# ApsaraDB/galaxysql

Hardware: NVIDIA H100
Metric: joined+aggregated rows/sec; achieved HBM GB/s vs peak, at 1/2/4/8 H100 (higher is better)
Workload: dtype int64

## Files before the change

galaxysql_b200/csrc/join_fast.cuh:

```cuda
#pragma once

#include <cub/block/block_scan.cuh>
#include <cub/device/device_scan.cuh>

#include "common.cuh"

namespace fj {

constexpr unsigned long long KEY_EMPTY = 0x8000000000000000ULL;
constexpr int THREADS = 512;
constexpr int RPT = 4;
constexpr int TILE = THREADS * RPT;
constexpr int MAX_WORDS = 4;
constexpr int MAX_P = 1024;
constexpr int MAX_DISP = 4096;
enum { FL_SENTINEL = 0, FL_DUP = 1, FL_DISP = 2, FL_NULLOUT = 3, FL_SPILL = 4, FL_COUNT = 5 };

struct Layout {
    int32_t nwords, ncols, key_col, key_i32;
    int32_t word[GSQL_MAX_COLS];
    int32_t half[GSQL_MAX_COLS];
};

static bool make_layout(const int32_t *types, int ncols, int key_col, Layout *L) {
    memset(L, 0, sizeof(*L));
    L->ncols = ncols;
    L->key_col = key_col;
    L->key_i32 = types[key_col] == GSQL_T_INT32;
    int next = 1;
    int open_word = -1;
    for (int c = 0; c < ncols; c++) {
        if (c == key_col) {
            L->word[c] = 0;
            L->half[c] = L->key_i32 ? 0 : 2;
            continue;
        }
        if (types[c] == GSQL_T_INT32) {
            if (open_word >= 0) {
                L->word[c] = open_word;
                L->half[c] = 1;
                open_word = -1;
            } else {
                L->word[c] = next;
                L->half[c] = 0;
                open_word = next++;
            }
        } else {
            L->word[c] = next++;
            L->half[c] = 2;
        }
    }
    L->nwords = next;
    return next <= MAX_WORDS;
}

__device__ __forceinline__ uint64_t key_hash(unsigned long long k) { return (k ^ (k >> 32)) * 0x9E3779B97F4A7C15ULL; }

template <int W>
__device__ __forceinline__ void pack_row(const DColSet &cols, const Layout &L, int64_t r, unsigned long long (&w)[W]) {
#pragma unroll
    for (int i = 0; i < W; i++) w[i] = 0;
#pragma unroll 1
    for (int c = 0; c < L.ncols; c++) {
        const DCol &col = cols.c[c];
        unsigned long long v;
        if (col.type == GSQL_T_INT32) {
            int x = ld_stream_4(reinterpret_cast<const int *>(col.data) + r);
            v = c == L.key_col ? (unsigned long long)(long long)x : (unsigned long long)(unsigned)x;
        } else {
            v = (unsigned long long)ld_stream_8(reinterpret_cast<const long long *>(col.data) + r);
        }
        int wi = L.word[c];
        if (L.half[c] == 1) v <<= 32;
#pragma unroll
        for (int i = 0; i < W; i++)
            if (i == wi) w[i] |= v;
    }
}

template <int W, int NC>
__device__ __forceinline__ void pack_tile_nc(const DColSet &cols, const Layout &L, int64_t base, int64_t limit, unsigned long long (&w)[RPT][W]) {
    unsigned long long v[NC > 0 ? NC : 1][RPT];
#pragma unroll
    for (int c = 0; c < NC; c++) {
        const DCol &col = cols.c[c];
        const bool is32 = col.type == GSQL_T_INT32;
#pragma unroll
        for (int k = 0; k < RPT; k++) {
            int64_t r = base + k * THREADS;
            v[c][k] = 0;
            if (r < limit) {
                if (is32) v[c][k] = (unsigned long long)(unsigned)ld_stream_4(reinterpret_cast<const int *>(col.data) + r);
                else v[c][k] = (unsigned long long)ld_stream_8(reinterpret_cast<const long long *>(col.data) + r);
            }
        }
    }
#pragma unroll
    for (int k = 0; k < RPT; k++)
#pragma unroll
        for (int i = 0; i < W; i++) w[k][i] = 0;
#pragma unroll
    for (int c = 0; c < NC; c++) {
        const bool sext = c == L.key_col && cols.c[c].type == GSQL_T_INT32;
        const int wi = L.word[c];
        const int sh = L.half[c] == 1 ? 32 : 0;
#pragma unroll
        for (int k = 0; k < RPT; k++) {
            unsigned long long vv = sext ? (unsigned long long)(long long)(int)(unsigned)v[c][k] : v[c][k];
            vv <<= sh;
#pragma unroll
            for (int i = 0; i < W; i++)
                if (i == wi) w[k][i] |= vv;
        }
    }
}

template <int W>
__device__ __forceinline__ void pack_tile_generic(const DColSet &cols, const Layout &L, int64_t base, int64_t limit, unsigned long long (&w)[RPT][W]) {
#pragma unroll
    for (int k = 0; k < RPT; k++)
#pragma unroll
        for (int i = 0; i < W; i++) w[k][i] = 0;
#pragma unroll 1
    for (int c = 0; c < L.ncols; c++) {
        const DCol &col = cols.c[c];
        const bool is32 = col.type == GSQL_T_INT32, iskey = c == L.key_col;
        const int wi = L.word[c];
        const int sh = L.half[c] == 1 ? 32 : 0;
        unsigned long long v[RPT];
#pragma unroll
        for (int k = 0; k < RPT; k++) {
            int64_t r = base + k * THREADS;
            v[k] = 0;
            if (r < limit) {
                if (is32) {
                    int x = ld_stream_4(reinterpret_cast<const int *>(col.data) + r);
                    v[k] = iskey ? (unsigned long long)(long long)x : (unsigned long long)(unsigned)x;
                } else {
                    v[k] = (unsigned long long)ld_stream_8(reinterpret_cast<const long long *>(col.data) + r);
                }
            }
        }
#pragma unroll
        for (int k = 0; k < RPT; k++) {
            unsigned long long vv = v[k] << sh;
#pragma unroll
            for (int i = 0; i < W; i++)
                if (i == wi) w[k][i] |= vv;
        }
    }
}

template <int W>
__device__ __forceinline__ void pack_tile(const DColSet &cols, const Layout &L, int64_t base, int64_t limit, unsigned long long (&w)[RPT][W]) {
    switch (L.ncols) {
    case 1: pack_tile_nc<W, 1>(cols, L, base, limit, w); break;
    case 2: pack_tile_nc<W, 2>(cols, L, base, limit, w); break;
    case 3: pack_tile_nc<W, 3>(cols, L, base, limit, w); break;
    case 4: pack_tile_nc<W, 4>(cols, L, base, limit, w); break;
    default: pack_tile_generic<W>(cols, L, base, limit, w); break;
    }
}

__device__ __forceinline__ unsigned long long load_key(const DCol &col, int64_t r) {
    if (col.type == GSQL_T_INT32) return (unsigned long long)(long long)ld_stream_4(reinterpret_cast<const int *>(col.data) + r);
    return (unsigned long long)ld_stream_8(reinterpret_cast<const long long *>(col.data) + r);
}

__device__ __forceinline__ unsigned int part_of(uint64_t h, int P) { return __umulhi((unsigned int)(h >> 32), (unsigned int)P); }

struct PartGeom {
    int64_t rows, chunk;
    int32_t P, nblocks;
};

template <int NT>
__global__ void __launch_bounds__(NT) k_fj_hist(DCol keycol, PartGeom g, int64_t *__restrict__ hist, int32_t *flags) {
    extern __shared__ unsigned int sh_hist[];
    for (int i = threadIdx.x; i < g.P; i += NT) sh_hist[i] = 0;
    __syncthreads();
    int64_t r0 = (int64_t)blockIdx.x * g.chunk;
    int64_t r1 = r0 + g.chunk < g.rows ? r0 + g.chunk : g.rows;
    bool sentinel = false;
    for (int64_t t0 = r0; t0 < r1; t0 += NT * RPT) {
        unsigned long long key[RPT];
#pragma unroll
        for (int k = 0; k < RPT; k++) {
            int64_t r = t0 + k * NT + threadIdx.x;
            key[k] = r < r1 ? load_key(keycol, r) : 0;
        }
#pragma unroll
        for (int k = 0; k < RPT; k++) {
            int64_t r = t0 + k * NT + threadIdx.x;
            if (r < r1) {
                sentinel |= key[k] == KEY_EMPTY;
                atomicAdd(&sh_hist[part_of(key_hash(key[k]), g.P)], 1u);
            }
        }
    }
    if (sentinel) flags[FL_SENTINEL] = 1;
    __syncthreads();
    for (int i = threadIdx.x; i < g.P; i += NT) hist[(int64_t)i * g.nblocks + blockIdx.x] = sh_hist[i];
}

__device__ __forceinline__ void cp_async_4(void *smem_dst, const void *gsrc) {
    asm volatile("cp.async.ca.shared.global [%0], [%1], 4;" ::"r"((uint32_t)__cvta_generic_to_shared(smem_dst)), "l"(gsrc) : "memory");
}
__device__ __forceinline__ void cp_async_8(void *smem_dst, const void *gsrc) {
    asm volatile("cp.async.ca.shared.global [%0], [%1], 8;" ::"r"((uint32_t)__cvta_generic_to_shared(smem_dst)), "l"(gsrc) : "memory");
}
__device__ __forceinline__ void cp_async_16(void *smem_dst, const void *gsrc) {
    asm volatile("cp.async.cg.shared.global [%0], [%1], 16;" ::"r"((uint32_t)__cvta_generic_to_shared(smem_dst)), "l"(gsrc) : "memory");
}
__device__ __forceinline__ void cp_async_16_hint(void *smem_dst, const void *gsrc, uint64_t pol) {
    asm volatile("cp.async.cg.shared.global.L2::cache_hint [%0], [%1], 16, %2;" ::"r"((uint32_t)__cvta_generic_to_shared(smem_dst)), "l"(gsrc), "l"(pol)
                 : "memory");
}
__device__ __forceinline__ void cp_async_commit() { asm volatile("cp.async.commit_group;" ::: "memory"); }
template <int N>
__device__ __forceinline__ void cp_async_wait() { asm volatile("cp.async.wait_group %0;" ::"n"(N) : "memory"); }

__device__ __forceinline__ uint32_t smem_u32(const void *p) { return (uint32_t)__cvta_generic_to_shared(p); }
__device__ __forceinline__ void mbar_init(unsigned long long *bar, int count) {
    asm volatile("mbarrier.init.shared::cta.b64 [%0], %1;" ::"r"(smem_u32(bar)), "r"(count) : "memory");
}
__device__ __forceinline__ void mbar_expect_tx(unsigned long long *bar, uint32_t bytes) {
    asm volatile("mbarrier.arrive.expect_tx.shared::cta.b64 _, [%0], %1;" ::"r"(smem_u32(bar)), "r"(bytes) : "memory");
}
__device__ __forceinline__ void mbar_wait(unsigned long long *bar, uint32_t parity) {
    uint32_t done = 0;
    while (!done)
        asm volatile("{\n\t.reg .pred p;\n\tmbarrier.try_wait.parity.shared::cta.b64 p, [%1], %2;\n\tselp.u32 %0, 1, 0, p;\n\t}"
                     : "=r"(done) : "r"(smem_u32(bar)), "r"(parity) : "memory");
}
__device__ __forceinline__ uint64_t l2_policy_evict_first() {
    uint64_t pol;
    asm volatile("createpolicy.fractional.L2::evict_first.b64 %0, 1.0;" : "=l"(pol));
    return pol;
}
__device__ __forceinline__ void tma_load_1d(void *smem_dst, const void *gsrc, uint32_t bytes, unsigned long long *bar, uint64_t pol) {
    asm volatile("cp.async.bulk.shared::cluster.global.mbarrier::complete_tx::bytes.L2::cache_hint [%0], [%1], %2, [%3], %4;" ::"r"(smem_u32(smem_dst)),
                 "l"(gsrc), "r"(bytes), "r"(smem_u32(bar)), "l"(pol)
                 : "memory");
}

template <bool FULL>
__device__ __forceinline__ void tile_prefetch(const DColSet &cols, const Layout &L, int64_t t0, int n_tile, unsigned char *buf) {
    const unsigned tid = threadIdx.x;
    unsigned char *sp = buf + tid * 4u;
#pragma unroll 1
    for (int c = 0; c < L.ncols; c++) {
        const DCol &col = cols.c[c];
        if (col.type == GSQL_T_INT32) {
            const int *gp = reinterpret_cast<const int *>(col.data) + t0 + tid;
#pragma unroll
            for (int k = 0; k < RPT; k++)
                if (FULL || (int)(k * THREADS + tid) < n_tile) cp_async_4(sp + k * THREADS * 4, gp + k * THREADS);
            sp += TILE * 4;
        } else {
            const long long *gp = reinterpret_cast<const long long *>(col.data) + t0 + tid;
            unsigned char *sp8 = sp + tid * 4u;
#pragma unroll
            for (int k = 0; k < RPT; k++)
                if (FULL || (int)(k * THREADS + tid) < n_tile) cp_async_8(sp8 + k * THREADS * 8, gp + k * THREADS);
            sp += TILE * 8;
        }
    }
    cp_async_commit();
}

template <int W, bool FULL>
__device__ __forceinline__ void pack_tile_smem(const DColSet &cols, const Layout &L, int n_tile, const unsigned char *buf,
                                               unsigned long long (&w)[RPT][W]) {
#pragma unroll
    for (int k = 0; k < RPT; k++)
#pragma unroll
        for (int i = 0; i < W; i++) w[k][i] = 0;
    const unsigned tid = threadIdx.x;
    const unsigned char *sp = buf + tid * 4u;
#pragma unroll 1
    for (int c = 0; c < L.ncols; c++) {
        const bool is32 = cols.c[c].type == GSQL_T_INT32, iskey = c == L.key_col;
        const int wi = L.word[c];
        const int sh = L.half[c] == 1 ? 32 : 0;
        unsigned long long v[RPT];
        if (is32) {
#pragma unroll
            for (int k = 0; k < RPT; k++) {
                int x = (FULL || (int)(k * THREADS + tid) < n_tile) ? *reinterpret_cast<const int *>(sp + k * THREADS * 4) : 0;
                v[k] = iskey ? (unsigned long long)(long long)x : (unsigned long long)(unsigned)x;
            }
            sp += TILE * 4;
        } else {
            const unsigned char *sp8 = sp + tid * 4u;
#pragma unroll
            for (int k = 0; k < RPT; k++)
                v[k] = (FULL || (int)(k * THREADS + tid) < n_tile) ? *reinterpret_cast<const unsigned long long *>(sp8 + k * THREADS * 8) : 0ULL;
            sp += TILE * 8;
        }
#pragma unroll
        for (int i = 0; i < W; i++)
            if (i == wi) {
#pragma unroll
                for (int k = 0; k < RPT; k++) w[k][i] |= v[k] << sh;
            }
    }
}

template <int W, bool PIPE>
__global__ void __launch_bounds__(THREADS, 2) k_fj_scatter(const __grid_constant__ DColSet cols, const __grid_constant__ Layout L, PartGeom g,
                                                        const int64_t *__restrict__ offs, unsigned long long *__restrict__ out) {
    extern __shared__ __align__(16) unsigned char smem_raw[];
    unsigned long long *stage = reinterpret_cast<unsigned long long *>(smem_raw);
    unsigned long long *cur = stage + (size_t)TILE * W;
    unsigned long long *delta = cur + g.P;
    unsigned int *hist = reinterpret_cast<unsigned int *>(delta + g.P);
    unsigned int *start = hist + g.P;
    unsigned short *spid = reinterpret_cast<unsigned short *>(start + g.P);
    unsigned char *inbuf = reinterpret_cast<unsigned char *>(spid + TILE);
    typedef cub::BlockScan<unsigned int, THREADS> BlockScan;
    __shared__ typename BlockScan::TempStorage scan_tmp;

    for (int p = threadIdx.x; p < g.P; p += THREADS) {
        cur[p] = (unsigned long long)offs[(int64_t)p * g.nblocks + blockIdx.x];
        hist[p] = 0;
    }
    __syncthreads();
    int64_t r0 = (int64_t)blockIdx.x * g.chunk;
    int64_t r1 = r0 + g.chunk < g.rows ? r0 + g.chunk : g.rows;
    if (PIPE && r0 < r1) {
        if (r1 - r0 >= TILE) tile_prefetch<true>(cols, L, r0, TILE, inbuf);
        else tile_prefetch<false>(cols, L, r0, (int)(r1 - r0), inbuf);
    }
    int it = 0;
    for (int64_t t0 = r0; t0 < r1; t0 += TILE, it++) {
        unsigned long long w[RPT][W];
        unsigned int pid[RPT], rank[RPT];
        const int n_tile = (int)(r1 - t0 < TILE ? r1 - t0 : TILE);
        const bool full = n_tile == TILE;
        if (PIPE) {
            const int64_t left = r1 - (t0 + TILE);
            unsigned char *nbuf = inbuf + (size_t)((it + 1) & 1) * TILE * W * 8;
            if (left >= TILE) tile_prefetch<true>(cols, L, t0 + TILE, TILE, nbuf);
            else if (left > 0) tile_prefetch<false>(cols, L, t0 + TILE, (int)left, nbuf);
            else cp_async_commit();
            cp_async_wait<1>();
            const unsigned char *cbuf = inbuf + (size_t)(it & 1) * TILE * W * 8;
            if (full) pack_tile_smem<W, true>(cols, L, n_tile, cbuf, w);
            else pack_tile_smem<W, false>(cols, L, n_tile, cbuf, w);
        } else {
            pack_tile<W>(cols, L, t0 + threadIdx.x, r1, w);
        }
        if (full) {
#pragma unroll
            for (int k = 0; k < RPT; k++) {
                pid[k] = part_of(key_hash(w[k][0]), g.P);
                rank[k] = atomicAdd(&hist[pid[k]], 1u);
            }
        } else {
#pragma unroll
            for (int k = 0; k < RPT; k++) {
                pid[k] = 0xffffffffu;
                if ((int)(k * THREADS + threadIdx.x) < n_tile) {
                    pid[k] = part_of(key_hash(w[k][0]), g.P);
                    rank[k] = atomicAdd(&hist[pid[k]], 1u);
                }
            }
        }
        __syncthreads();
        {
            constexpr int IPT = MAX_P / THREADS;
            unsigned int v[IPT];
#pragma unroll
            for (int i = 0; i < IPT; i++) {
                int p = threadIdx.x * IPT + i;
                v[i] = p < g.P ? hist[p] : 0;
            }
            BlockScan(scan_tmp).ExclusiveSum(v, v);
#pragma unroll
            for (int i = 0; i < IPT; i++) {
                int p = threadIdx.x * IPT + i;
                if (p < g.P) {
                    start[p] = v[i];
                    unsigned long long c = cur[p];
                    delta[p] = c - v[i];
                    cur[p] = c + hist[p];
                    hist[p] = 0;
                }
            }
        }
        __syncthreads();
#pragma unroll
        for (int k = 0; k < RPT; k++) {
            if (full || pid[k] != 0xffffffffu) {
                unsigned int pos = start[pid[k]] + rank[k];
                if (W == 2) {
                    int4 v;
                    v.x = (int)(unsigned)w[k][0]; v.y = (int)(unsigned)(w[k][0] >> 32);
                    v.z = (int)(unsigned)w[k][W - 1]; v.w = (int)(unsigned)(w[k][W - 1] >> 32);
                    *reinterpret_cast<int4 *>(stage + (size_t)pos * 2) = v;
                } else {
#pragma unroll
                    for (int i = 0; i < W; i++) stage[(size_t)pos * W + i] = w[k][i];
                }
                spid[pos] = (unsigned short)pid[k];
            }
        }
        __syncthreads();
#pragma unroll
        for (int k = 0; k < RPT; k++) {
            const int i = k * THREADS + threadIdx.x;
            if (full || i < n_tile) {
                unsigned long long dst = delta[spid[i]] + (unsigned)i;
                if (W == 2) {
                    st_stream_16(out + dst * 2, *reinterpret_cast<const int4 *>(stage + (size_t)i * 2));
                } else {
#pragma unroll
                    for (int j = 0; j < W; j++) st_stream_8(out + dst * W + j, (long long)stage[(size_t)i * W + j]);
                }
            }
        }
        __syncthreads();
    }
}

template <int W>
__global__ void __launch_bounds__(THREADS, 2) k_fj_scatter_direct(const __grid_constant__ DColSet cols, const __grid_constant__ Layout L, PartGeom g,
                                                               const int64_t *__restrict__ offs, unsigned long long *__restrict__ out) {
    extern __shared__ __align__(16) unsigned char smem_raw[];
    unsigned long long *base = reinterpret_cast<unsigned long long *>(smem_raw);
    unsigned int *cnt = reinterpret_cast<unsigned int *>(base + g.P);
    for (int p = threadIdx.x; p < g.P; p += THREADS) {
        base[p] = (unsigned long long)offs[(int64_t)p * g.nblocks + blockIdx.x];
        cnt[p] = 0;
    }
    __syncthreads();
    const int64_t r0 = (int64_t)blockIdx.x * g.chunk;
    const int64_t r1 = r0 + g.chunk < g.rows ? r0 + g.chunk : g.rows;
    for (int64_t t0 = r0; t0 < r1; t0 += TILE) {
        unsigned long long w[RPT][W];
        pack_tile<W>(cols, L, t0 + threadIdx.x, r1, w);
#pragma unroll
        for (int k = 0; k < RPT; k++) {
            if (t0 + k * THREADS + threadIdx.x >= r1) continue;
            const unsigned int pid = part_of(key_hash(w[k][0]), g.P);
            const unsigned long long dst = base[pid] + atomicAdd(&cnt[pid], 1u);
            if (W == 2) {
                int4 v;
                v.x = (int)(unsigned)w[k][0]; v.y = (int)(unsigned)(w[k][0] >> 32);
                v.z = (int)(unsigned)w[k][W - 1]; v.w = (int)(unsigned)(w[k][W - 1] >> 32);
                *reinterpret_cast<int4 *>(out + dst * 2) = v;
            } else {
#pragma unroll
                for (int i = 0; i < W; i++) out[dst * W + i] = w[k][i];
            }
        }
    }
}

static size_t scatter_smem_bytes(int W, int P, bool pipe) {
    return (size_t)TILE * W * 8 + (size_t)P * 8 * 2 + (size_t)P * 4 * 2 + (size_t)TILE * 2 + (pipe ? (size_t)2 * TILE * W * 8 : 0);
}

constexpr int SM_THREADS = 1024;
__host__ __device__ constexpr int sm_rpt_max(int W) { return W == 1 ? 8 : W == 2 ? 6 : W == 3 ? 4 : 3; }

static size_t scatter_sm_smem_bytes(int W, int P, int rpt) {
    const size_t T = (size_t)SM_THREADS * rpt;
    return T * W * 8 * 2 + (size_t)P * (8 * 3 + 4 * 3) + T * 2;
}

struct Regions {
    unsigned long long *fill;
    int64_t cap;
    int32_t K;
};

template <int W>
__global__ void __launch_bounds__(SM_THREADS, 1) k_fj_scatter_sm(const __grid_constant__ DColSet cols, const __grid_constant__ Layout L, PartGeom g,
                                                                 int rpt, const int64_t *__restrict__ offs, Regions RG,
                                                                 unsigned long long *__restrict__ out, int32_t *flags) {
    constexpr int R = sm_rpt_max(W);
    const int T = SM_THREADS * rpt;
    extern __shared__ __align__(128) unsigned char smem_raw[];
    unsigned long long *stage = reinterpret_cast<unsigned long long *>(smem_raw);
    unsigned char *inbuf = reinterpret_cast<unsigned char *>(stage + (size_t)T * W);
    unsigned long long *cur = reinterpret_cast<unsigned long long *>(inbuf + (size_t)T * W * 8);
    unsigned long long *delta = cur + g.P;
    unsigned long long *delta2 = delta + g.P;
    unsigned int *hist = reinterpret_cast<unsigned int *>(delta2 + g.P);
    unsigned int *start = hist + g.P;
    unsigned int *split = start + g.P;
    unsigned short *spid = reinterpret_cast<unsigned short *>(split + g.P);
    __shared__ __align__(8) unsigned long long bar;
    __shared__ int spill;
    typedef cub::BlockScan<unsigned int, SM_THREADS, cub::BLOCK_SCAN_WARP_SCANS> BlockScan;
    __shared__ typename BlockScan::TempStorage scan_tmp;
    const int tid = threadIdx.x, lane = tid & 31, warp = tid >> 5;

    uint32_t bulk_bytes = 0, my_off = 0, off = 0;
    bool my_bulk = false;
    for (int c = 0; c < L.ncols; c++) {
        const uint32_t bytes = (uint32_t)T * (cols.c[c].type == GSQL_T_INT32 ? 4u : 8u);
        const bool aligned = ((uintptr_t)cols.c[c].data & 15) == 0;
        if (c == warp) { my_off = off; my_bulk = aligned; }
        off += bytes;
        if (aligned) bulk_bytes += bytes;
    }
    const bool issuer = lane == 0 && warp < L.ncols && my_bulk;
    uint64_t pol = 0;
    if (issuer) pol = l2_policy_evict_first();

    if (tid == 0) {
        mbar_init(&bar, 1);
        asm volatile("fence.mbarrier_init.release.cluster;" ::: "memory");
        spill = 0;
    }
    static_assert(MAX_P <= SM_THREADS, "one partition per thread");
    const unsigned long long K = (unsigned long long)RG.K;
    unsigned long long nxt = 0;
    if (tid < g.P) {
        if (K) {
            const unsigned long long r = atomicAdd(&RG.fill[tid], 2 * K);
            if (r + 2 * K > (unsigned long long)RG.cap) spill = 1;
            cur[tid] = (unsigned long long)tid * RG.cap + r;
            nxt = r + K;
        } else {
            cur[tid] = (unsigned long long)offs[(int64_t)tid * g.nblocks + blockIdx.x];
        }
        hist[tid] = 0;
    }
    __syncthreads();
    if (spill) {
        if (tid == 0) flags[FL_SPILL] = 1;
        return;
    }
    const int64_t r0 = (int64_t)blockIdx.x * g.chunk;
    const int64_t r1 = r0 + g.chunk < g.rows ? r0 + g.chunk : g.rows;

    auto load_tile = [&](int64_t t0, int n_tile) {
        const bool full = n_tile == T;
        if (full && bulk_bytes) {
            if (tid == 0) mbar_expect_tx(&bar, bulk_bytes);
            if (issuer) {
                const DCol &col = cols.c[warp];
                const uint32_t width = col.type == GSQL_T_INT32 ? 4u : 8u;
                tma_load_1d(inbuf + my_off, reinterpret_cast<const unsigned char *>(col.data) + t0 * width, (uint32_t)T * width, &bar, pol);
            }
        }
        unsigned char *sp = inbuf;
#pragma unroll 1
        for (int c = 0; c < L.ncols; c++) {
            const DCol &col = cols.c[c];
            const bool is32 = col.type == GSQL_T_INT32;
            if (!(full && ((uintptr_t)col.data & 15) == 0)) {
#pragma unroll
                for (int k = 0; k < R; k++) {
                    const int e = k * SM_THREADS + tid;
                    if (k < rpt && e < n_tile) {
                        if (is32) cp_async_4(sp + e * 4, reinterpret_cast<const int *>(col.data) + t0 + e);
                        else cp_async_8(sp + e * 8, reinterpret_cast<const long long *>(col.data) + t0 + e);
                    }
                }
            }
            sp += (size_t)T * (is32 ? 4 : 8);
        }
        cp_async_commit();
    };

    uint32_t phase = 0;
    if (r0 < r1) load_tile(r0, (int)(r1 - r0 < T ? r1 - r0 : T));
    for (int64_t t0 = r0; t0 < r1; t0 += T) {
        const int n_tile = (int)(r1 - t0 < T ? r1 - t0 : T);
        if (n_tile == T && bulk_bytes) {
            mbar_wait(&bar, phase);
            phase ^= 1u;
        }
        cp_async_wait<0>();
        unsigned long long w[R][W];
#pragma unroll
        for (int k = 0; k < R; k++)
#pragma unroll
            for (int i = 0; i < W; i++) w[k][i] = 0;
        {
            const unsigned char *sp = inbuf;
#pragma unroll 1
            for (int c = 0; c < L.ncols; c++) {
                const bool is32 = cols.c[c].type == GSQL_T_INT32, iskey = c == L.key_col;
                const int wi = L.word[c];
                const int sh = L.half[c] == 1 ? 32 : 0;
#pragma unroll
                for (int k = 0; k < R; k++) {
                    const int e = k * SM_THREADS + tid;
                    if (k < rpt && e < n_tile) {
                        unsigned long long v;
                        if (is32) {
                            const int x = *reinterpret_cast<const int *>(sp + e * 4);
                            v = iskey ? (unsigned long long)(long long)x : (unsigned long long)(unsigned)x;
                        } else {
                            v = *reinterpret_cast<const unsigned long long *>(sp + e * 8);
                        }
#pragma unroll
                        for (int i = 0; i < W; i++)
                            if (i == wi) w[k][i] |= v << sh;
                    }
                }
                sp += (size_t)T * (is32 ? 4 : 8);
            }
        }
        unsigned int pr[R];
#pragma unroll
        for (int k = 0; k < R; k++) {
            pr[k] = 0xffffffffu;
            if (k < rpt && k * SM_THREADS + tid < n_tile) {
                const unsigned int pid = part_of(key_hash(w[k][0]), g.P);
                pr[k] = (pid << 16) | atomicAdd(&hist[pid], 1u);
                if (K && w[k][0] == KEY_EMPTY) flags[FL_SPILL] = 1;
            }
        }
        __syncthreads();
        const bool more = t0 + T < r1;
        const int n_next = more ? (int)(r1 - (t0 + T) < T ? r1 - (t0 + T) : T) : 0;
        if (more) load_tile(t0 + T, n_next);
        {
            const int p = tid;
            unsigned int v = p < g.P ? hist[p] : 0;
            BlockScan(scan_tmp).ExclusiveSum(v, v);
            if (p < g.P) {
                start[p] = v;
                const unsigned int h = hist[p];
                const unsigned long long c = cur[p];
                delta[p] = c - v;
                split[p] = v + h;
                cur[p] = c + h;
                const unsigned int room = K ? (unsigned int)(K - (c & (K - 1))) : 0xffffffffu;
                if (h >= room) {
                    const unsigned long long rest = h - room;
                    unsigned long long b, span = K;
                    if (rest < K) {
                        b = nxt;
                        nxt = atomicAdd(&RG.fill[p], K);
                    } else {
                        span = (rest / K + 1) * K;
                        b = atomicAdd(&RG.fill[p], span);
                    }
                    if (b + span > (unsigned long long)RG.cap) {
                        spill = 1;
                        flags[FL_SPILL] = 1;
                    }
                    const unsigned long long base = (unsigned long long)p * RG.cap + b;
                    split[p] = v + room;
                    delta2[p] = base - (v + room);
                    cur[p] = base + rest;
                }
                hist[p] = 0;
            }
        }
        __syncthreads();
        if (spill) {
            if (more && n_next == T && bulk_bytes) mbar_wait(&bar, phase);
            cp_async_wait<0>();
            return;
        }
#pragma unroll
        for (int k = 0; k < R; k++) {
            if (pr[k] != 0xffffffffu) {
                const unsigned int pid = pr[k] >> 16;
                const unsigned int pos = start[pid] + (pr[k] & 0xffffu);
                if (W == 2) {
                    int4 v;
                    v.x = (int)(unsigned)w[k][0]; v.y = (int)(unsigned)(w[k][0] >> 32);
                    v.z = (int)(unsigned)w[k][W - 1]; v.w = (int)(unsigned)(w[k][W - 1] >> 32);
                    *reinterpret_cast<int4 *>(stage + (size_t)pos * 2) = v;
                } else {
#pragma unroll
                    for (int i = 0; i < W; i++) stage[(size_t)pos * W + i] = w[k][i];
                }
                spid[pos] = (unsigned short)pid;
            }
        }
        __syncthreads();
#pragma unroll
        for (int k = 0; k < R; k++) {
            const int i = k * SM_THREADS + tid;
            if (k < rpt && i < n_tile) {
                const unsigned int p = spid[i];
                const unsigned long long dst = ((unsigned)i < split[p] ? delta[p] : delta2[p]) + (unsigned)i;
                if (W == 2) {
                    st_stream_16(out + dst * 2, *reinterpret_cast<const int4 *>(stage + (size_t)i * 2));
                } else {
#pragma unroll
                    for (int j = 0; j < W; j++) st_stream_8(out + dst * W + j, (long long)stage[(size_t)i * W + j]);
                }
            }
        }
    }
    if (K) {
        __syncthreads();
        if (tid < g.P) delta2[tid] = nxt;
        __syncthreads();
        for (int p = warp; p < g.P; p += SM_THREADS / 32) {
            const unsigned long long c = cur[p], e = (c | (K - 1)) + 1;
            const unsigned long long base = (unsigned long long)p * RG.cap, n0 = delta2[p];
            const unsigned long long n1 = n0 + K < (unsigned long long)RG.cap ? n0 + K : (unsigned long long)RG.cap;
            for (unsigned long long r = c + lane; r < e; r += 32) st_stream_8(out + r * W, (long long)KEY_EMPTY);
            for (unsigned long long r = base + n0 + lane; r < base + n1; r += 32) st_stream_8(out + r * W, (long long)KEY_EMPTY);
        }
    }
}

__global__ void __launch_bounds__(256) k_fj_region_tail(Regions RG, int W, unsigned long long *out) {
    const unsigned long long p = blockIdx.x, cap = (unsigned long long)RG.cap, f = RG.fill[p];
    for (unsigned long long r = p * cap + (f < cap ? f : cap) + threadIdx.x; r < (p + 1) * cap; r += 256)
        st_stream_8(out + r * W, (long long)KEY_EMPTY);
}

template <int W>
__global__ void __launch_bounds__(THREADS) k_fj_table_init(unsigned long long *table, uint64_t nslots) {
    for (uint64_t i = blockIdx.x * (uint64_t)blockDim.x + threadIdx.x; i < nslots; i += (uint64_t)gridDim.x * blockDim.x) {
        table[i * W] = KEY_EMPTY;
#pragma unroll
        for (int j = 1; j < W; j++) table[i * W + j] = 0;
    }
}

template <int W>
__global__ void __launch_bounds__(THREADS, 2) k_fj_insert(const unsigned long long *__restrict__ packed, const __grid_constant__ DColSet cols,
                                                       const __grid_constant__ Layout L, int64_t n, unsigned long long *table, uint64_t nslots,
                                                       int32_t *flags, const unsigned long long *n_dev) {
    if (n_dev && *n_dev < (unsigned long long)n) n = (int64_t)*n_dev;
    for (int64_t t0 = (int64_t)blockIdx.x * TILE; t0 < n; t0 += (int64_t)gridDim.x * TILE) {
        unsigned long long w[RPT][W];
        if (packed) {
#pragma unroll
            for (int k = 0; k < RPT; k++) {
                int64_t r = t0 + k * THREADS + threadIdx.x;
#pragma unroll
                for (int i = 0; i < W; i++) w[k][i] = r < n ? (unsigned long long)ld_stream_8(packed + r * W + i) : 0;
            }
        } else {
            pack_tile<W>(cols, L, t0 + threadIdx.x, n, w);
        }
        uint64_t sl[RPT];
        unsigned long long prev[RPT];
        bool pending[RPT];
        bool any = false;
#pragma unroll
        for (int k = 0; k < RPT; k++) {
            int64_t r = t0 + k * THREADS + threadIdx.x;
            sl[k] = __umul64hi(key_hash(w[k][0]), nslots);
            pending[k] = r < n;
            if (pending[k] && w[k][0] == KEY_EMPTY) { flags[FL_SENTINEL] = 1; pending[k] = false; }
            any |= pending[k];
        }
        int disp = 0;
        while (__any_sync(0xffffffffu, any)) {
#pragma unroll
            for (int k = 0; k < RPT; k++)
                if (pending[k]) prev[k] = atomicCAS(table + sl[k] * W, KEY_EMPTY, w[k][0]);
            any = false;
#pragma unroll
            for (int k = 0; k < RPT; k++) {
                if (!pending[k]) continue;
                if (prev[k] == KEY_EMPTY) {
#pragma unroll
                    for (int i = 1; i < W; i++) table[sl[k] * W + i] = w[k][i];
                    pending[k] = false;
                } else if (prev[k] == w[k][0]) {
                    flags[FL_DUP] = 1;
                    pending[k] = false;
                } else {
                    if (++sl[k] == nslots) sl[k] = 0;
                }
                any |= pending[k];
            }
            if (++disp > MAX_DISP) { if (any) flags[FL_DISP] = 1; break; }
        }
    }
}

constexpr int BS_THREADS = 512;
constexpr int BS_WIN = 2048;
__host__ __device__ constexpr int bs_rpt(int W) { return 12 / W; }

template <int W>
__device__ __forceinline__ void load_row(const unsigned long long *p, unsigned long long (&w)[W]) {
    if (W == 2) {
        const int4 v = ld_stream_16(p);
        w[0] = ((unsigned long long)(unsigned)v.y << 32) | (unsigned)v.x;
        w[W - 1] = ((unsigned long long)(unsigned)v.w << 32) | (unsigned)v.z;
    } else {
#pragma unroll
        for (int i = 0; i < W; i++) w[i] = (unsigned long long)ld_stream_8(p + i);
    }
}

template <int W>
__device__ __forceinline__ void defer_row(const unsigned long long (&w)[W], unsigned long long *def, unsigned long long *ndef, int64_t def_cap,
                                          int32_t *flags) {
    const unsigned long long pos = atomicAdd(ndef, 1ULL);
    if (pos < (unsigned long long)def_cap) {
#pragma unroll
        for (int i = 0; i < W; i++) def[pos * W + i] = w[i];
    } else {
        flags[FL_DISP] = 1;
    }
}

static size_t split_smem_bytes(int W) { return (size_t)BS_THREADS * bs_rpt(W) * (W * 8 + 2); }

template <int W>
__global__ void __launch_bounds__(BS_THREADS) k_fj_build_split(const unsigned long long *__restrict__ packed, int64_t rows, int64_t chunk, int P,
                                                                  uint64_t spp, uint64_t nslots, int lgB, unsigned long long *table, unsigned int *fill,
                                                                  unsigned long long *def, unsigned long long *ndef, int64_t def_cap, int32_t *flags) {
    constexpr int R = bs_rpt(W), T = BS_THREADS * R, IPT = BS_WIN / BS_THREADS;
    extern __shared__ __align__(16) unsigned char smem_raw[];
    unsigned long long *stage = reinterpret_cast<unsigned long long *>(smem_raw);
    unsigned short *sb = reinterpret_cast<unsigned short *>(stage + (size_t)T * W);
    __shared__ unsigned int cnt[BS_WIN], start[BS_WIN], base[BS_WIN];
    __shared__ unsigned long long s_blo;
    __shared__ unsigned int s_nwin;
    typedef cub::BlockScan<unsigned int, BS_THREADS> BlockScan;
    __shared__ typename BlockScan::TempStorage scan_tmp;
    const int tid = threadIdx.x;
    const int64_t r0 = (int64_t)blockIdx.x * chunk;
    const int64_t r1 = r0 + chunk < rows ? r0 + chunk : rows;
    for (int i = tid; i < BS_WIN; i += BS_THREADS) cnt[i] = 0;
    if (tid == 0) {
        const uint64_t pa = part_of(key_hash(packed[r0 * W]), P), pb = part_of(key_hash(packed[(r1 - 1) * W]), P);
        uint64_t s_hi = (pb + 2) * spp;
        if (s_hi > nslots) s_hi = nslots;
        const uint64_t blo = (pa * spp) >> lgB, bhi = ((s_hi - 1) >> lgB) + 1;
        s_blo = blo;
        s_nwin = (unsigned)(bhi - blo < (uint64_t)BS_WIN ? bhi - blo : BS_WIN);
    }
    __syncthreads();
    const uint64_t blo = s_blo;
    const unsigned nwin = s_nwin;
    for (int64_t t0 = r0; t0 < r1; t0 += T) {
        const int n_tile = (int)(r1 - t0 < T ? r1 - t0 : T);
        unsigned long long w[R][W];
        unsigned int br[R], n_staged;
#pragma unroll
        for (int k = 0; k < R; k++)
            if (k * BS_THREADS + tid < n_tile) load_row<W>(packed + (t0 + k * BS_THREADS + tid) * W, w[k]);
#pragma unroll
        for (int k = 0; k < R; k++) {
            br[k] = 0xffffffffu;
            if (k * BS_THREADS + tid >= n_tile) continue;
            const uint64_t rel = (__umul64hi(key_hash(w[k][0]), nslots) >> lgB) - blo;
            if (rel < nwin) {
                br[k] = ((unsigned)rel << 16) | atomicAdd(&cnt[rel], 1u);
            } else {
                defer_row<W>(w[k], def, ndef, def_cap, flags);
            }
        }
        __syncthreads();
        {
            unsigned int v[IPT];
#pragma unroll
            for (int i = 0; i < IPT; i++) v[i] = cnt[tid * IPT + i];
            unsigned int c[IPT];
#pragma unroll
            for (int i = 0; i < IPT; i++) c[i] = v[i];
            BlockScan(scan_tmp).ExclusiveSum(v, v, n_staged);
#pragma unroll
            for (int i = 0; i < IPT; i++) {
                const unsigned e = tid * IPT + i;
                start[e] = v[i];
                if (c[i]) {
                    base[e] = atomicAdd(&fill[blo + e], c[i]);
                    cnt[e] = 0;
                }
            }
        }
        __syncthreads();
#pragma unroll
        for (int k = 0; k < R; k++) {
            if (br[k] == 0xffffffffu) continue;
            const unsigned pos = start[br[k] >> 16] + (br[k] & 0xffffu);
#pragma unroll
            for (int i = 0; i < W; i++) stage[(size_t)pos * W + i] = w[k][i];
            sb[pos] = (unsigned short)(br[k] >> 16);
        }
        __syncthreads();
        for (int i = tid; i < (int)n_staged; i += BS_THREADS) {
            const unsigned e = sb[i];
            const uint64_t s0 = (blo + e) << lgB;
            const uint64_t cap = nslots - s0 < (1ull << lgB) ? nslots - s0 : (1ull << lgB);
            const uint64_t pos = (uint64_t)base[e] + (unsigned)i - start[e];
            unsigned long long rw[W];
#pragma unroll
            for (int j = 0; j < W; j++) rw[j] = stage[(size_t)i * W + j];
            if (pos >= cap) { defer_row<W>(rw, def, ndef, def_cap, flags); continue; }
            unsigned long long *dst = table + (s0 + pos) * W;
            if (W == 2) {
                int4 v;
                v.x = (int)(unsigned)rw[0]; v.y = (int)(unsigned)(rw[0] >> 32);
                v.z = (int)(unsigned)rw[W - 1]; v.w = (int)(unsigned)(rw[W - 1] >> 32);
                *reinterpret_cast<int4 *>(dst) = v;
            } else {
#pragma unroll
                for (int j = 0; j < W; j++) dst[j] = rw[j];
            }
        }
    }
}

template <int W>
__global__ void __launch_bounds__(BS_THREADS) k_fj_build_slab(unsigned long long *table, uint64_t nslots, int lgB, const unsigned int *__restrict__ fill,
                                                              unsigned long long *def, unsigned long long *ndef, int64_t def_cap, int32_t *flags) {
    constexpr int R = bs_rpt(W) < 8 ? bs_rpt(W) : 8;
    extern __shared__ __align__(16) unsigned long long st[];
    const int tid = threadIdx.x;
    const uint64_t s0 = (uint64_t)blockIdx.x << lgB;
    const unsigned cap = (unsigned)(nslots - s0 < (1ull << lgB) ? nslots - s0 : (1ull << lgB));
    const unsigned n = fill[blockIdx.x] < cap ? fill[blockIdx.x] : cap;
    unsigned long long *g = table + s0 * W;
    for (unsigned i = tid; i < cap; i += BS_THREADS) {
        st[(size_t)i * W] = KEY_EMPTY;
#pragma unroll
        for (int j = 1; j < W; j++) st[(size_t)i * W + j] = 0;
    }
    __syncthreads();
    for (unsigned i0 = 0; i0 < n; i0 += BS_THREADS * R) {
        unsigned long long w[R][W];
#pragma unroll
        for (int k = 0; k < R; k++) {
            const unsigned i = i0 + k * BS_THREADS + tid;
            if (i < n) load_row<W>(g + (size_t)i * W, w[k]);
        }
#pragma unroll
        for (int k = 0; k < R; k++) {
            if (i0 + k * BS_THREADS + tid >= n) continue;
            const unsigned long long key = w[k][0];
            if (key == KEY_EMPTY) { flags[FL_SENTINEL] = 1; continue; }
            unsigned s = (unsigned)(__umul64hi(key_hash(key), nslots) - s0);
            int disp = 0;
            while (true) {
                if (s >= cap) { defer_row<W>(w[k], def, ndef, def_cap, flags); break; }
                const unsigned long long prev = atomicCAS(&st[(size_t)s * W], KEY_EMPTY, key);
                if (prev == KEY_EMPTY) {
#pragma unroll
                    for (int i = 1; i < W; i++) st[(size_t)s * W + i] = w[k][i];
                    break;
                }
                if (prev == key) { flags[FL_DUP] = 1; break; }
                ++s;
                if (++disp > MAX_DISP) { flags[FL_DISP] = 1; break; }
            }
        }
    }
    __syncthreads();
    const unsigned nw = cap * W;
    const int4 *s4 = reinterpret_cast<const int4 *>(st);
    for (unsigned i = tid; i < nw / 2; i += BS_THREADS) st_stream_16(g + (size_t)i * 2, s4[i]);
    if ((nw & 1) && tid == 0) st_stream_8(g + nw - 1, (long long)st[nw - 1]);
}

struct OutMap {
    void *data[GSQL_MAX_COLS * 2];
    uint8_t *nulls[GSQL_MAX_COLS * 2];
    int8_t side[GSQL_MAX_COLS * 2];
    int8_t word[GSQL_MAX_COLS * 2];
    int8_t half[GSQL_MAX_COLS * 2];
    int8_t is32[GSQL_MAX_COLS * 2];
    int32_t nout;
    int32_t join_type;
    int32_t stage_off[GSQL_MAX_COLS * 2];
    int32_t stage_null_off[GSQL_MAX_COLS * 2];
    int32_t stage_bytes;
    int32_t lookup_mode;
};

template <int W>
__device__ __forceinline__ unsigned long long pick(const unsigned long long (&w)[W], int idx) {
    unsigned long long v = w[0];
#pragma unroll
    for (int i = 1; i < W; i++)
        if (i == idx) v = w[i];
    return v;
}


template <int R, int PW, int BP, int J, int H>
__device__ __forceinline__ void write_col(char *data, uint8_t *nulls, bool null_if_unmatched, const unsigned long long (&pw)[R][PW],
                                          const unsigned long long (&bp)[R][BP], const bool (&found)[R], const bool (&em)[R],
                                          const unsigned long long (&pos)[R], int32_t *flags) {
#pragma unroll
    for (int k = 0; k < R; k++) {
        if (!em[k]) continue;
        unsigned long long v = J < PW ? pw[k][J < PW ? J : 0] : bp[k][(J >= PW && J - PW < BP) ? J - PW : 0];
        const bool isnull = null_if_unmatched && !found[k];
        if (isnull) v = 0;
        if (nulls) nulls[pos[k]] = isnull ? 1 : 0;
        else if (isnull) flags[FL_NULLOUT] = 1;
        if (H == 0) st_stream_4(data + pos[k] * 4, (int)(unsigned)v);
        else if (H == 1) st_stream_4(data + pos[k] * 4, (int)(unsigned)(v >> 32));
        else st_stream_8(data + pos[k] * 8, (long long)v);
    }
}

template <int R, int PW, int BP>
__device__ __forceinline__ void stage_words(char *staging, int tile_rows, bool want_flags, const unsigned long long (&pw)[R][PW],
                                            const unsigned long long (&bp)[R][BP], const bool (&found)[R], const bool (&em)[R],
                                            const unsigned int (&li)[R]) {
    unsigned long long *sw = reinterpret_cast<unsigned long long *>(staging);
    uint8_t *sf = reinterpret_cast<uint8_t *>(staging) + (size_t)(PW + BP) * tile_rows * 8;
#pragma unroll
    for (int k = 0; k < R; k++) {
        if (!em[k]) continue;
// ... 477 lines not shown
```

Measured before the change: 23.27 billion.

## Double-buffer scatter input tiles and flush partitions with TMA bulk stores

Reworks the single-SM partition scatter kernel so the input staging buffer is double-buffered with two mbarriers, prefetching the tile two steps ahead, and the staging area reuses the consumed input buffer. For even word widths, each partition's contiguous run in shared memory is written to global memory with one TMA bulk store per thread instead of per-row streaming stores. Column packing moves into a helper with full-tile specialisations that drop bounds checks. This aims to overlap loads with compute and cut store instruction count. In exchange it adds async-proxy fences, waits on bulk-store reads each tile, and puts per-partition store issue onto at most P threads, which could serialise on small or skewed partitions.

```diff
diff --git a/galaxysql_b200/csrc/join_fast.cuh b/galaxysql_b200/csrc/join_fast.cuh
--- a/galaxysql_b200/csrc/join_fast.cuh
+++ b/galaxysql_b200/csrc/join_fast.cuh
@@ -2,6 +2,7 @@
 
 #include <cub/block/block_scan.cuh>
 #include <cub/device/device_scan.cuh>
+#include <type_traits>
 
 #include "common.cuh"
 
@@ -233,6 +234,15 @@
         asm volatile("{\n\t.reg .pred p;\n\tmbarrier.try_wait.parity.shared::cta.b64 p, [%1], %2;\n\tselp.u32 %0, 1, 0, p;\n\t}"
                      : "=r"(done) : "r"(smem_u32(bar)), "r"(parity) : "memory");
 }
+__device__ __forceinline__ void tma_store_1d(void *gdst, const void *smem_src, uint32_t bytes, uint64_t pol) {
+    asm volatile("cp.async.bulk.global.shared::cta.bulk_group.L2::cache_hint [%0], [%1], %2, %3;" ::"l"(gdst), "r"(smem_u32(smem_src)),
+                 "r"(bytes), "l"(pol)
+                 : "memory");
+}
+__device__ __forceinline__ void tma_store_commit() { asm volatile("cp.async.bulk.commit_group;" ::: "memory"); }
+__device__ __forceinline__ void tma_store_wait_read() { asm volatile("cp.async.bulk.wait_group.read 0;" ::: "memory"); }
+__device__ __forceinline__ void tma_store_wait() { asm volatile("cp.async.bulk.wait_group 0;" ::: "memory"); }
+__device__ __forceinline__ void fence_proxy_async_smem() { asm volatile("fence.proxy.async.shared::cta;" ::: "memory"); }
 __device__ __forceinline__ uint64_t l2_policy_evict_first() {
     uint64_t pol;
     asm volatile("createpolicy.fractional.L2::evict_first.b64 %0, 1.0;" : "=l"(pol));
@@ -470,6 +480,51 @@
     return T * W * 8 * 2 + (size_t)P * (8 * 3 + 4 * 3) + T * 2;
 }
 
+template <int W, int R, bool FULL>
+__device__ __forceinline__ void pack_tile_sm(const DColSet &cols, const Layout &L, int rpt, int n_tile, int T, const unsigned char *buf,
+                                             unsigned long long (&w)[R][W]) {
+#pragma unroll
+    for (int k = 0; k < R; k++)
+#pragma unroll
+        for (int i = 0; i < W; i++) w[k][i] = 0;
+    const int tid = threadIdx.x;
+    const unsigned char *sp = buf;
+#pragma unroll 1
+    for (int c = 0; c < L.ncols; c++) {
+        const bool is32 = cols.c[c].type == GSQL_T_INT32;
+        unsigned long long v[R];
+        if (is32) {
+            const int *p = reinterpret_cast<const int *>(sp) + tid;
+            int x[R];
+#pragma unroll
+            for (int k = 0; k < R; k++) x[k] = (FULL || (k < rpt && k * SM_THREADS + tid < n_tile)) ? p[k * SM_THREADS] : 0;
+            if (c == L.key_col) {
+#pragma unroll
+                for (int k = 0; k < R; k++) v[k] = (unsigned long long)(long long)x[k];
+            } else if (L.half[c] == 1) {
+#pragma unroll
+                for (int k = 0; k < R; k++) v[k] = (unsigned long long)(unsigned)x[k] << 32;
+            } else {
+#pragma unroll
+                for (int k = 0; k < R; k++) v[k] = (unsigned long long)(unsigned)x[k];
+            }
+            sp += (size_t)T * 4;
+        } else {
+            const unsigned long long *p = reinterpret_cast<const unsigned long long *>(sp) + tid;
+#pragma unroll
+            for (int k = 0; k < R; k++) v[k] = (FULL || (k < rpt && k * SM_THREADS + tid < n_tile)) ? p[k * SM_THREADS] : 0ULL;
+            sp += (size_t)T * 8;
+        }
+        const int wi = L.word[c];
+#pragma unroll
+        for (int i = 0; i < W; i++)
+            if (i == wi) {
+#pragma unroll
+                for (int k = 0; k < R; k++) w[k][i] |= v[k];
+            }
+    }
+}
+
 struct Regions {
     unsigned long long *fill;
     int64_t cap;
@@ -483,16 +538,14 @@
     constexpr int R = sm_rpt_max(W);
     const int T = SM_THREADS * rpt;
     extern __shared__ __align__(128) unsigned char smem_raw[];
-    unsigned long long *stage = reinterpret_cast<unsigned long long *>(smem_raw);
-    unsigned char *inbuf = reinterpret_cast<unsigned char *>(stage + (size_t)T * W);
-    unsigned long long *cur = reinterpret_cast<unsigned long long *>(inbuf + (size_t)T * W * 8);
+    unsigned long long *cur = reinterpret_cast<unsigned long long *>(smem_raw + (size_t)T * W * 8 * 2);
     unsigned long long *delta = cur + g.P;
     unsigned long long *delta2 = delta + g.P;
     unsigned int *hist = reinterpret_cast<unsigned int *>(delta2 + g.P);
     unsigned int *start = hist + g.P;
     unsigned int *split = start + g.P;
     unsigned short *spid = reinterpret_cast<unsigned short *>(split + g.P);
-    __shared__ __align__(8) unsigned long long bar;
+    __shared__ __align__(8) unsigned long long bar[2];
     __shared__ int spill;
     typedef cub::BlockScan<unsigned int, SM_THREADS, cub::BLOCK_SCAN_WARP_SCANS> BlockScan;
     __shared__ typename BlockScan::TempStorage scan_tmp;
@@ -510,9 +563,12 @@
     const bool issuer = lane == 0 && warp < L.ncols && my_bulk;
     uint64_t pol = 0;
     if (issuer) pol = l2_policy_evict_first();
+    constexpr bool BULK_FLUSH = W % 2 == 0;
+    const uint64_t spol = BULK_FLUSH && tid < g.P ? l2_policy_evict_first() : 0;
 
     if (tid == 0) {
-        mbar_init(&bar, 1);
+        mbar_init(&bar[0], 1);
+        mbar_init(&bar[1], 1);
         asm volatile("fence.mbarrier_init.release.cluster;" ::: "memory");
         spill = 0;
     }
@@ -538,14 +594,17 @@
     const int64_t r0 = (int64_t)blockIdx.x * g.chunk;
     const int64_t r1 = r0 + g.chunk < g.rows ? r0 + g.chunk : g.rows;
 
-    auto load_tile = [&](int64_t t0, int n_tile) {
+    auto tile_rows = [&](int64_t t0) { return t0 < r1 ? (int)(r1 - t0 < T ? r1 - t0 : T) : 0; };
+    auto tile_bulk = [&](int n_tile) { return n_tile == T && bulk_bytes != 0; };
+    auto load_tile = [&](int64_t t0, int n_tile, int b) {
+        unsigned char *const inbuf = smem_raw + (size_t)b * T * W * 8;
         const bool full = n_tile == T;
-        if (full && bulk_bytes) {
-            if (tid == 0) mbar_expect_tx(&bar, bulk_bytes);
+        if (tile_bulk(n_tile)) {
+            if (tid == 0) mbar_expect_tx(&bar[b], bulk_bytes);
             if (issuer) {
                 const DCol &col = cols.c[warp];
                 const uint32_t width = col.type == GSQL_T_INT32 ? 4u : 8u;
-                tma_load_1d(inbuf + my_off, reinterpret_cast<const unsigned char *>(col.data) + t0 * width, (uint32_t)T * width, &bar, pol);
+                tma_load_1d(inbuf + my_off, reinterpret_cast<const unsigned char *>(col.data) + t0 * width, (uint32_t)T * width, &bar[b], pol);
             }
         }
         unsigned char *sp = inbuf;
@@ -569,45 +628,22 @@
     };
 
     uint32_t phase = 0;
-    if (r0 < r1) load_tile(r0, (int)(r1 - r0 < T ? r1 - r0 : T));
-    for (int64_t t0 = r0; t0 < r1; t0 += T) {
-        const int n_tile = (int)(r1 - t0 < T ? r1 - t0 : T);
-        if (n_tile == T && bulk_bytes) {
-            mbar_wait(&bar, phase);
-            phase ^= 1u;
-        }
-        cp_async_wait<0>();
+    load_tile(r0, tile_rows(r0), 0);
+    load_tile(r0 + T, tile_rows(r0 + T), 1);
+    int b = 0;
+    for (int64_t t0 = r0; t0 < r1; t0 += T, b ^= 1) {
+        const int n_tile = tile_rows(t0);
+        unsigned char *const tbuf = smem_raw + (size_t)b * T * W * 8;
+        unsigned long long *const stage = reinterpret_cast<unsigned long long *>(tbuf);
+        if (tile_bulk(n_tile)) {
+            mbar_wait(&bar[b], (phase >> b) & 1u);
+            phase ^= 1u << b;
+        }
+        cp_async_wait<1>();
+        const bool full = n_tile == T && rpt == R;
         unsigned long long w[R][W];
-#pragma unroll
-        for (int k = 0; k < R; k++)
-#pragma unroll
-            for (int i = 0; i < W; i++) w[k][i] = 0;
-        {
-            const unsigned char *sp = inbuf;
-#pragma unroll 1
-            for (int c = 0; c < L.ncols; c++) {
-                const bool is32 = cols.c[c].type == GSQL_T_INT32, iskey = c == L.key_col;
-                const int wi = L.word[c];
-                const int sh = L.half[c] == 1 ? 32 : 0;
-#pragma unroll
-                for (int k = 0; k < R; k++) {
-                    const int e = k * SM_THREADS + tid;
-                    if (k < rpt && e < n_tile) {
-                        unsigned long long v;
-                        if (is32) {
-                            const int x = *reinterpret_cast<const int *>(sp + e * 4);
-                            v = iskey ? (unsigned long long)(long long)x : (unsigned long long)(unsigned)x;
-                        } else {
-                            v = *reinterpret_cast<const unsigned long long *>(sp + e * 8);
-                        }
-#pragma unroll
-                        for (int i = 0; i < W; i++)
-                            if (i == wi) w[k][i] |= v << sh;
-                    }
-                }
-                sp += (size_t)T * (is32 ? 4 : 8);
-            }
-        }
+        if (full) pack_tile_sm<W, R, true>(cols, L, rpt, n_tile, T, tbuf, w);
+        else pack_tile_sm<W, R, false>(cols, L, rpt, n_tile, T, tbuf, w);
         unsigned int pr[R];
 #pragma unroll
         for (int k = 0; k < R; k++) {
@@ -619,9 +655,6 @@
             }
         }
         __syncthreads();
-        const bool more = t0 + T < r1;
-        const int n_next = more ? (int)(r1 - (t0 + T) < T ? r1 - (t0 + T) : T) : 0;
-        if (more) load_tile(t0 + T, n_next);
         {
             const int p = tid;
             unsigned int v = p < g.P ? hist[p] : 0;
@@ -658,8 +691,9 @@
         }
         __syncthreads();
         if (spill) {
-            if (more && n_next == T && bulk_bytes) mbar_wait(&bar, phase);
+            if (tile_bulk(tile_rows(t0 + T))) mbar_wait(&bar[b ^ 1], (phase >> (b ^ 1)) & 1u);
             cp_async_wait<0>();
+            if (BULK_FLUSH) tma_store_wait();
             return;
         }
 #pragma unroll
@@ -676,27 +710,47 @@
 #pragma unroll
                     for (int i = 0; i < W; i++) stage[(size_t)pos * W + i] = w[k][i];
                 }
-                spid[pos] = (unsigned short)pid;
-            }
-        }
+                if (!BULK_FLUSH) spid[pos] = (unsigned short)pid;
+            }
+        }
+        if (BULK_FLUSH) fence_proxy_async_smem();
         __syncthreads();
-#pragma unroll
-        for (int k = 0; k < R; k++) {
-            const int i = k * SM_THREADS + tid;
-            if (k < rpt && i < n_tile) {
-                const unsigned int p = spid[i];
-                const unsigned long long dst = ((unsigned)i < split[p] ? delta[p] : delta2[p]) + (unsigned)i;
-                if (W == 2) {
-                    st_stream_16(out + dst * 2, *reinterpret_cast<const int4 *>(stage + (size_t)i * 2));
-                } else {
-#pragma unroll
-                    for (int j = 0; j < W; j++) st_stream_8(out + dst * W + j, (long long)stage[(size_t)i * W + j]);
+        if (BULK_FLUSH) {
+            if (tid < g.P) {
+                const unsigned int s = start[tid], e = tid + 1 < g.P ? start[tid + 1] : (unsigned)n_tile, m = split[tid] < e ? split[tid] : e;
+                if (m > s) tma_store_1d(out + (delta[tid] + s) * W, stage + (size_t)s * W, (m - s) * W * 8, spol);
+                if (e > m) tma_store_1d(out + (delta2[tid] + m) * W, stage + (size_t)m * W, (e - m) * W * 8, spol);
+                tma_store_commit();
+                tma_store_wait_read();
+            }
+        }
+        auto flush = [&](auto all_rows) {
+#pragma unroll
+            for (int k = 0; k < R; k++) {
+                const int i = k * SM_THREADS + tid;
+                if (decltype(all_rows)::value || (k < rpt && i < n_tile)) {
+                    const unsigned int p = spid[i];
+                    const unsigned long long dst = ((unsigned)i < split[p] ? delta[p] : delta2[p]) + (unsigned)i;
+                    if (W == 2) {
+                        st_stream_16(out + dst * 2, *reinterpret_cast<const int4 *>(stage + (size_t)i * 2));
+                    } else {
+#pragma unroll
+                        for (int j = 0; j < W; j++) st_stream_8(out + dst * W + j, (long long)stage[(size_t)i * W + j]);
+                    }
                 }
             }
-        }
+        };
+        if (!BULK_FLUSH) {
+            if (full) flush(std::true_type{});
+            else flush(std::false_type{});
+        }
+        const int64_t t2 = t0 + 2 * (int64_t)T;
+        const int n2 = tile_rows(t2);
+        if (tile_bulk(n2)) fence_proxy_async_smem();
+        __syncthreads();
+        load_tile(t2, n2, b);
     }
     if (K) {
-        __syncthreads();
         if (tid < g.P) delta2[tid] = nxt;
         __syncthreads();
         for (int p = warp; p < g.P; p += SM_THREADS / 32) {
@@ -707,6 +761,7 @@
             for (unsigned long long r = base + n0 + lane; r < base + n1; r += 32) st_stream_8(out + r * W, (long long)KEY_EMPTY);
         }
     }
+    if (BULK_FLUSH) tma_store_wait();
 }
 
 __global__ void __launch_bounds__(256) k_fj_region_tail(Regions RG, int W, unsigned long long *out) {
```

Measured after the change: 23.35 billion, median of 6. About the same (+0.3%).
